# AntoineBlanot/LC2IS

Measured on AMD Instinct MI355X. Metric: training-step images/sec (512x512, ADE20K-150), higher is better.
Workload: dtype bf16; 1 GPU; BaseModelWithText ViT-B/16 + CLIP-text + decoder + fused head/CE train step, 512x512, 151 classes, text len 16, sgd; batch_per_gpu=32, global_batch=32, parallelism=dp1

## Files before the change

### include/lc2is_hip.h

```cpp
#ifndef LC2IS_HIP_H
#define LC2IS_HIP_H
#include <stddef.h>
#include <stdint.h>

#ifdef __cplusplus
extern "C" {
#endif

#define LC2IS_ACT_NONE 0
#define LC2IS_ACT_QUICK_GELU 1
#define LC2IS_ACT_RELU 2
#define LC2IS_ACT_DQUICK_GELU 3
#define LC2IS_ACT_DRELU 4
#define LC2IS_ACT_QUICK_GELU_GRAD 5
#define LC2IS_ACT_MUL_AUX 6
#define LC2IS_ACT_GELU_ERF 7
#define LC2IS_ACT_DGELU_ERF 8
#define LC2IS_ACT_ADD_AUX 9

#define LC2IS_INTERP_BICUBIC 0
#define LC2IS_INTERP_BILINEAR 1

typedef void* lc2is_stream_t;

typedef struct {
  const void* src;
  void* dst;
  void* dstT;
  int N, K, ld_dst, ld_dstT;
  int tile_start;
  int flags;
} lc2is_shadow_desc;

const char* lc2is_version(void);

int lc2is_set_cu_budget(int ncu);
int lc2is_get_cu_budget(void);

int lc2is_gemm_nt_bf16(const void* A, int lda, const void* W, int ldw, const float* bias,
                       const float* resid, int ldr, const void* aux_in, int ldx, void* out_bf16, int ldo,
                       float* out_f32, int ldf, void* aux_out, int ldy, int M, int N, int K, int act,
                       int tile_cfg, lc2is_stream_t stream);

size_t lc2is_gemm_nt_ln_xchg_bytes(int M, int N);
int lc2is_gemm_nt_ln_bf16(const void* A, int lda, const void* W, int ldw, const float* bias, const float* resid, int ldr,
                          float* out_f32, int ldf, const float* gamma, const float* beta, float eps, void* ln_out, int ldl,
                          float* mean, float* rstd, void* xchg, size_t xchg_bytes, int M, int N, int K, lc2is_stream_t stream);

int lc2is_gemm_nt_bf16_batched(const void* A, int lda, long stride_a, const void* W, int ldw, long stride_w,
                               void* out_bf16, int ldo, long stride_ob, float* out_f32, int ldf, long stride_of,
                               int M, int N, int K, int batch, lc2is_stream_t stream);

size_t lc2is_gemm_tn_workspace_bytes(int M, int N, int K);
int lc2is_gemm_tn_bf16(const void* dY, int ldy, const void* X, int ldx, float* dW, int ldw, float* db, int M,
                       int N, int K, int accumulate, void* workspace, size_t workspace_bytes,
                       lc2is_stream_t stream);

#define LC2IS_TN_GROUP_MAX 128
typedef struct lc2is_tn_problem {
  const void* dY; const void* X; float* dW; float* db;
  int ldy, ldx, ldw, M, N, K, accumulate;
} lc2is_tn_problem;
size_t lc2is_gemm_tn_grouped_workspace_bytes(const lc2is_tn_problem* problems, int n);
int lc2is_gemm_tn_grouped(const lc2is_tn_problem* problems, int n, void* workspace, size_t workspace_bytes,
                          lc2is_stream_t stream);
int lc2is_release_captured_tables(void);
int lc2is_captured_tables_mark(void);
int lc2is_release_captured_tables_range(int first, int last);

size_t lc2is_colsum_workspace_bytes(int M, int N);
int lc2is_colsum_bf16(const void* dY, int ldy, float* db, int M, int N, int accumulate, void* workspace,
                      size_t workspace_bytes, lc2is_stream_t stream);

int lc2is_layernorm_fwd(const void* x, int ldx, int x_is_bf16, const float* gamma, const float* beta, void* y_bf16,
                        int ldy, float* y_f32, int ldyf, float* mean, float* rstd, int M, int C, float eps,
                        lc2is_stream_t stream);

size_t lc2is_layernorm_bwd_workspace_bytes(int M, int C);
int lc2is_layernorm_bwd(const void* dy_bf16, int lddy, const float* dy_f32, int lddyf, const void* x,
                        int ldx, int x_is_bf16, const float* gamma, const float* mean, const float* rstd,
                        const void* dres, int lddres, int dres_is_bf16, float* dx_f32, int lddx, void* dx_bf16,
                        int lddxb, float* dgamma, float* dbeta, int accumulate, int M, int C, void* workspace,
                        size_t workspace_bytes, lc2is_stream_t stream);

#define LC2IS_LN_PARTIALS_MAX 64
typedef struct {
  const float* partials;
  float* dgamma;
  float* dbeta;
  int nparts;
  int C;
  int accumulate;
} lc2is_ln_partials;
int lc2is_layernorm_bwd_partials(int M, int C);
int lc2is_ln_partials_reduce(const lc2is_ln_partials* items, int n, lc2is_stream_t stream);

int lc2is_attention_fwd(const void* Q, int ldq, const void* K, int ldk, const void* V, int ldv, void* O,
                        int ldo, float* lse2, const float* kbias, int B, int H, int Sq, int Sk, int D,
                        float scale, int causal, lc2is_stream_t stream);

int lc2is_attention_bwd(const void* Q, int ldq, const void* K, int ldk, const void* V, int ldv,
                        const void* O, int ldo, const void* dO, int lddo, void* dQ, int lddq, void* dK,
                        int lddk, void* dV, int lddv, const float* lse2, float* delta, const float* kbias,
                        int B, int H, int Sq, int Sk, int D, float scale, int causal, lc2is_stream_t stream);

int lc2is_attention_fwd_dropout(const void* Q, int ldq, const void* K, int ldk, const void* V, int ldv, void* O,
                                int ldo, float* lse2, const float* kbias, int B, int H, int Sq, int Sk, int D,
                                float scale, int causal, float p_drop, unsigned long long seed, lc2is_stream_t stream);
int lc2is_attention_bwd_dropout(const void* Q, int ldq, const void* K, int ldk, const void* V, int ldv,
                                const void* O, int ldo, const void* dO, int lddo, void* dQ, int lddq, void* dK,
                                int lddk, void* dV, int lddv, const float* lse2, float* delta, const float* kbias,
                                int B, int H, int Sq, int Sk, int D, float scale, int causal, float p_drop,
                                unsigned long long seed, lc2is_stream_t stream);

int lc2is_dropout_rows_f32(const float* x, int ldx, const float* resid, int ldr, float* y32, int ldy, void* y16,
                           int ldy16, int M, int C, int rows_per_sample, float p, unsigned long long seed,
                           lc2is_stream_t stream);
int lc2is_dropout_rows_bf16(const void* x, int ldx, void* y, int ldy, int M, int C, float p, unsigned long long seed,
                            lc2is_stream_t stream);
int lc2is_dropout_mask(unsigned char* out, long rows, int cols, float p, unsigned long long seed, lc2is_stream_t stream);


int lc2is_shadow_refresh(const lc2is_shadow_desc* descs, int ndesc, int total_tiles, lc2is_stream_t stream);
int lc2is_cast_f32_bf16(const float* src, int ld_src, void* dst_bf16, int ld_dst, int M, int C,
                        lc2is_stream_t stream);
int lc2is_transpose_bf16(const void* src, int ld_src, void* dst, int ld_dst, int R, int C,
                         lc2is_stream_t stream);
int lc2is_transpose_bf16_batched(const void* src, int ld_src, long stride_src, void* dst, int ld_dst, long stride_dst,
                                 int R, int C, int batch, lc2is_stream_t stream);

int lc2is_patchify(const float* pixels, void* out_bf16, int ld_out, int B, int H, int W, int patch,
                   lc2is_stream_t stream);
int lc2is_vit_embed_fwd(const float* patch, int ld_patch, const float* cls, const float* pos, float* x,
                        int ldx, int B, int P, int C, lc2is_stream_t stream);
int lc2is_vit_embed_bwd(const float* dx, int ldx, float* dpos, float* dcls, void* dpatch_bf16, int ld_dpatch,
                        int B, int P, int C, int accumulate, lc2is_stream_t stream);
int lc2is_text_embed_fwd(const int64_t* ids, const float* tok, const float* pos, float* x, int ldx, int B,
                         int L, int C, int vocab, lc2is_stream_t stream);
int lc2is_text_embed_bwd(const int64_t* ids, const float* dx, int ldx, float* dtok, float* dpos, int B, int L,
                         int C, int vocab, int accumulate, lc2is_stream_t stream);
int lc2is_rows_copy_f32(const float* src, int S_src, int src_off, float* dst_f32, void* dst_bf16, int S_dst,
                        int dst_off, int B, int n, int C, lc2is_stream_t stream);
int lc2is_rows_copy_bf16(const void* src, int S_src, int src_off, float* dst_f32, void* dst_bf16, int S_dst,
                         int dst_off, int B, int n, int C, lc2is_stream_t stream);

int lc2is_sgd_step(float* params, const float* grads, float* momentum_buf, size_t n, float lr, float momentum,
                   float weight_decay, float grad_scale, lc2is_stream_t stream);
int lc2is_adamw_step(float* params, const float* grads, float* exp_avg, float* exp_avg_sq, size_t n, float lr,
                     float beta1, float beta2, float eps, float weight_decay, int step, float grad_scale,
                     lc2is_stream_t stream);

size_t lc2is_head_upsample_ce_workspace_bytes(int B, int h, int w, int C, int S, int mode, int want_grad);
int lc2is_head_upsample_ce(const float* scores_lo, int ld, const int64_t* labels, float* dscores_lo,
                           float* scores_hi, float* loss_sum, int B, int h, int w, int C, int S, int mode,
                           long ignore_index, float grad_scale, void* workspace, size_t workspace_bytes,
                           lc2is_stream_t stream);
int lc2is_head_upsample_ce_opts(const float* scores_lo, int ld, const int64_t* labels, float* dscores_lo,
                                float* scores_hi, float* loss_sum, int B, int h, int w, int C, int S, int mode,
                                long ignore_index, float grad_scale, const float* class_weight, float label_smoothing,
                                void* workspace, size_t workspace_bytes, lc2is_stream_t stream);
int lc2is_upsample_bwd_nchw(const float* dhi, float* dlo, int ld, int B, int h, int w, int C, int S, int mode,
                            lc2is_stream_t stream);
int lc2is_ce_nchw_fwd(const float* logits, const int64_t* labels, float* lse, float* loss_sum, int B, int C,
                      long HW, long ignore_index, lc2is_stream_t stream);
int lc2is_ce_nchw_bwd(const float* logits, const int64_t* labels, const float* lse, const float* grad_scale_dev,
                      float grad_scale, float* dlogits, int B, int C, long HW, long ignore_index,
                      lc2is_stream_t stream);
int lc2is_ce_nchw_fwd_opts(const float* logits, const int64_t* labels, float* lse, float* loss_sum, float* loss_px,
                           int B, int C, long HW, long ignore_index, const float* class_weight, float label_smoothing,
                           lc2is_stream_t stream);
int lc2is_ce_nchw_bwd_opts(const float* logits, const int64_t* labels, const float* lse, const float* grad_scale_dev,
                           float grad_scale, const float* grad_px, float* dlogits, int B, int C, long HW,
                           long ignore_index, const float* class_weight, float label_smoothing,
                           lc2is_stream_t stream);
size_t lc2is_ce_nchw_fwd_workspace_bytes(int B, long HW);
int lc2is_ce_nchw_fwd_ordered(const float* logits, const int64_t* labels, float* lse, float* loss_sum, float* loss_px,
                              int B, int C, long HW, long ignore_index, const float* class_weight, float label_smoothing,
// ... 139 lines not shown
```

### lc2is_amd/csrc/layernorm.hip

```cpp
#include "common.h"
#include "lc2is_hip.h"
#include <cstdlib>

namespace {

#ifndef LN_BWD_OCC
#define LN_BWD_OCC 4
#endif
constexpr int LN_MAXV = 8;

__device__ __forceinline__ float4 load_bf16x4(const bf16_t* p) {
  const uint2 pk = *reinterpret_cast<const uint2*>(p);
  return make_float4(bf16_to_f32((bf16_t)(pk.x & 0xffff)), bf16_to_f32((bf16_t)(pk.x >> 16)),
                     bf16_to_f32((bf16_t)(pk.y & 0xffff)), bf16_to_f32((bf16_t)(pk.y >> 16)));
}

template <int NV>
__global__ __launch_bounds__(256) void ln_fwd_kernel(const float* __restrict__ x, const bf16_t* __restrict__ xb, int ldx,
                                                      const float* __restrict__ gamma,
                                                      const float* __restrict__ beta, bf16_t* y, int ldy,
                                                      float* yf, int ldyf, float* mean_out, float* rstd_out,
                                                      int M, int C, float eps) {
  const int lane = threadIdx.x & 63;
  const int C4 = C >> 2;
  float4 gm[NV], bt[NV];
#pragma unroll
  for (int i = 0; i < NV; ++i) {
    const int c4 = lane + 64 * i;
    gm[i] = (c4 < C4) ? reinterpret_cast<const float4*>(gamma)[c4] : make_float4(0.f, 0.f, 0.f, 0.f);
    bt[i] = (beta && c4 < C4) ? reinterpret_cast<const float4*>(beta)[c4] : make_float4(0.f, 0.f, 0.f, 0.f);
  }
  const int stride = gridDim.x * 4;
  int row = blockIdx.x * 4 + (threadIdx.x >> 6);
  if (row >= M) return;
  auto load_row = [&](int r, float4 (&dst)[NV]) __attribute__((always_inline)) {
    if (xb) {
#pragma unroll
      for (int i = 0; i < NV; ++i) {
        const int c4 = lane + 64 * i;
        dst[i] = (c4 < C4) ? load_bf16x4(xb + (size_t)r * ldx + 4 * c4) : make_float4(0.f, 0.f, 0.f, 0.f);
      }
      return;
    }
    const float4* xr = reinterpret_cast<const float4*>(x + (size_t)r * ldx);
#pragma unroll
    for (int i = 0; i < NV; ++i) {
      const int c4 = lane + 64 * i;
      dst[i] = (c4 < C4) ? xr[c4] : make_float4(0.f, 0.f, 0.f, 0.f);
    }
  };
  float4 v[NV], nx[NV];
  load_row(row, v);
  for (; row < M; row += stride) {
    const bool more = row + stride < M;
    if (more) load_row(row + stride, nx);
    float s = 0.f;
#pragma unroll
    for (int i = 0; i < NV; ++i) {
      const int c4 = lane + 64 * i;
      if (c4 < C4) s += (v[i].x + v[i].y) + (v[i].z + v[i].w);
    }
    const float mean = wave_sum(s) / (float)C;
    float q = 0.f;
#pragma unroll
    for (int i = 0; i < NV; ++i) {
      const int c4 = lane + 64 * i;
      if (c4 < C4) {
        const float a = v[i].x - mean, b = v[i].y - mean, c = v[i].z - mean, d = v[i].w - mean;
        q += (a * a + b * b) + (c * c + d * d);
      }
    }
    const float rstd = rsqrtf(wave_sum(q) / (float)C + eps);
    if (lane == 0) {
      if (mean_out) mean_out[row] = mean;
      if (rstd_out) rstd_out[row] = rstd;
    }
#pragma unroll
    for (int i = 0; i < NV; ++i) {
      const int c4 = lane + 64 * i;
      if (c4 < C4) {
        float4 o;
        o.x = (v[i].x - mean) * rstd * gm[i].x;
        o.y = (v[i].y - mean) * rstd * gm[i].y;
        o.z = (v[i].z - mean) * rstd * gm[i].z;
// ... 123 lines not shown
    for (int c = threadIdx.x; c < 2 * C; c += 256) ws[(size_t)rz * 2 * C + c] = 0.f;
  float4 gm[NV], dg[NV], db[NV];
#pragma unroll
  for (int i = 0; i < NV; ++i) {
    const int c4 = lane + 64 * i;
    gm[i] = (c4 < C4) ? reinterpret_cast<const float4*>(gamma)[c4] : make_float4(0.f, 0.f, 0.f, 0.f);
    dg[i] = make_float4(0.f, 0.f, 0.f, 0.f);
    db[i] = make_float4(0.f, 0.f, 0.f, 0.f);
  }
  struct Raw { uint2 dy[NV], rv[NV]; f32x4_t xf[XB ? 1 : NV]; uint2 xb[XB ? NV : 1]; };
  auto load_row = [&](int row, Raw& r) __attribute__((always_inline)) {
#pragma unroll
    for (int i = 0; i < NV; ++i) {
      const int c4 = lane + 64 * i;
      const bool ok = c4 < C4;
      r.rv[i] = (dresb && ok) ? *reinterpret_cast<const uint2*>(dresb + (size_t)row * lddres + 4 * c4) : make_uint2(0u, 0u);
      r.dy[i] = ok ? *reinterpret_cast<const uint2*>(dyb + (size_t)row * lddy + 4 * c4) : make_uint2(0u, 0u);
      if constexpr (XB) r.xb[i] = ok ? *reinterpret_cast<const uint2*>((const bf16_t*)xv_ + (size_t)row * ldx + 4 * c4) : make_uint2(0u, 0u);
      else r.xf[i] = ok ? __builtin_nontemporal_load(reinterpret_cast<const f32x4_t*>((const float*)xv_ + (size_t)row * ldx + 4 * c4))
                        : f32x4_t{0.f, 0.f, 0.f, 0.f};
    }
  };
  auto widen = [](uint2 pk) {
    return make_float4(bf16_to_f32((bf16_t)(pk.x & 0xffff)), bf16_to_f32((bf16_t)(pk.x >> 16)),
                       bf16_to_f32((bf16_t)(pk.y & 0xffff)), bf16_to_f32((bf16_t)(pk.y >> 16)));
  };
  const int stride = gridDim.x * 4;
  int row = blockIdx.x * 4 + wave;
  Raw cur, nxt;
  if (row < M) load_row(row, cur);
  for (; row < M; row += stride) {
    const bool more = row + stride < M;
    if (more) load_row(row + stride, nxt);
    const float mu = mean[row], rs = rstd[row];
    float4 xh[NV], dy[NV];
    float s1 = 0.f, s2 = 0.f;
#pragma unroll
    for (int i = 0; i < NV; ++i) {
      const int c4 = lane + 64 * i;
      if (c4 < C4) {
        float4 xv;
        if constexpr (XB) xv = widen(cur.xb[i]);
        else xv = make_float4(cur.xf[i][0], cur.xf[i][1], cur.xf[i][2], cur.xf[i][3]);
        dy[i] = widen(cur.dy[i]);
        xh[i] = make_float4((xv.x - mu) * rs, (xv.y - mu) * rs, (xv.z - mu) * rs, (xv.w - mu) * rs);
        const float a = dy[i].x * gm[i].x, b = dy[i].y * gm[i].y, c = dy[i].z * gm[i].z, d = dy[i].w * gm[i].w;
        s1 += (a + b) + (c + d);
        s2 += (a * xh[i].x + b * xh[i].y) + (c * xh[i].z + d * xh[i].w);
        dg[i].x += dy[i].x * xh[i].x; dg[i].y += dy[i].y * xh[i].y;
        dg[i].z += dy[i].z * xh[i].z; dg[i].w += dy[i].w * xh[i].w;
        db[i].x += dy[i].x; db[i].y += dy[i].y; db[i].z += dy[i].z; db[i].w += dy[i].w;
      }
    }
    const float c1 = wave_sum(s1) / (float)C, c2 = wave_sum(s2) / (float)C;
#pragma unroll
    for (int i = 0; i < NV; ++i) {
      const int c4 = lane + 64 * i;
      if (c4 < C4) {
        const float4 rv = widen(cur.rv[i]);
        float4 o;
        o.x = rs * (dy[i].x * gm[i].x - c1 - xh[i].x * c2);
        o.y = rs * (dy[i].y * gm[i].y - c1 - xh[i].y * c2);
        o.z = rs * (dy[i].z * gm[i].z - c1 - xh[i].z * c2);
        o.w = rs * (dy[i].w * gm[i].w - c1 - xh[i].w * c2);
        o.x += rv.x; o.y += rv.y; o.z += rv.z; o.w += rv.w;
        uint2 pk = make_uint2(pack_bf16x2(o.x, o.y), pack_bf16x2(o.z, o.w));
        __builtin_nontemporal_store(i32x2_t{(int)pk.x, (int)pk.y}, reinterpret_cast<i32x2_t*>(dxb + (size_t)row * lddxb + 4 * c4));
      }
    }
    if (more) cur = nxt;
  }
  float* r = red;
#pragma unroll
  for (int pass = 0; pass < 2; ++pass) {
    __syncthreads();
#pragma unroll
    for (int i = 0; i < NV; ++i) {
      const int c4 = lane + 64 * i;
      if (c4 < C4) *reinterpret_cast<float4*>(r + wave * 2048 + 4 * c4) = pass ? db[i] : dg[i];
    }
    __syncthreads();
    for (int c = threadIdx.x; c < C; c += 256) {
      const float t = (r[c] + r[2048 + c]) + (r[4096 + c] + r[6144 + c]);
      ws[((size_t)blockIdx.x * 2 + pass) * C + c] = t;
    }
  }
}

__global__ __launch_bounds__(256) void ln_bwd_reduce_kernel(const float* __restrict__ ws, int nblk, int C,
                                                             float* dgamma, float* dbeta, int accumulate) {
  const int c = blockIdx.x * 256 + threadIdx.x;
  if (c >= C) return;
  float g = 0.f, b = 0.f;
  for (int k = 0; k < nblk; ++k) {
    g += ws[((size_t)k * 2 + 0) * C + c];
    b += ws[((size_t)k * 2 + 1) * C + c];
  }
  if (dgamma) dgamma[c] = accumulate ? dgamma[c] + g : g;
  if (dbeta) dbeta[c] = accumulate ? dbeta[c] + b : b;
}

inline int ln_bwd_blocks(int M, int C) {
  const int nv = (C / 4 + 63) / 64;
  const int cap = 256 * (nv <= 3 ? LN_BWD_OCC : nv == 4 ? 3 : nv <= 6 ? 2 : 1);
  int nb = (M + 3) / 4;
  return nb > cap ? cap : nb;
}

}

static int ln_fwd_blocks(int M) {
  static const int cap = getenv("LC2IS_LN_FWD_BLOCKS") ? atoi(getenv("LC2IS_LN_FWD_BLOCKS")) : 2048;
  const int need = (M + 3) / 4;
  return need < cap ? need : (cap > 0 ? cap : need);
}

extern "C" int lc2is_layernorm_fwd(const void* x, int ldx, int x_is_bf16, const float* gamma, const float* beta,
                                   void* y_bf16, int ldy, float* y_f32, int ldyf, float* mean, float* rstd,
                                   int M, int C, float eps, lc2is_stream_t stream_) {
  hipStream_t stream = (hipStream_t)stream_;
  if (!x || !gamma || (!y_bf16 && !y_f32)) return LC2IS_ERR_NULL;
  const float* xf = x_is_bf16 ? nullptr : (const float*)x;
  const bf16_t* xb = x_is_bf16 ? (const bf16_t*)x : nullptr;
  if (M <= 0 || C <= 0 || C % 4 || C > LN_MAXV * 256) return LC2IS_ERR_SHAPE;
  if (ldx < C || ldx % 4 || (y_bf16 && (ldy < C || ldy % 4)) || (y_f32 && (ldyf < C || ldyf % 4)))
    return LC2IS_ERR_SHAPE;
#define LN_FWD(NV_)                                                                                  \
  hipLaunchKernelGGL(ln_fwd_kernel<NV_>, dim3(ln_fwd_blocks(M)), dim3(256), 0, stream, xf, xb, ldx, gamma, beta, \
                     (bf16_t*)y_bf16, ldy, y_f32, ldyf, mean, rstd, M, C, eps)
  const int nv = (C / 4 + 63) / 64;
  if (nv <= 1) LN_FWD(1); else if (nv == 2) LN_FWD(2); else if (nv == 3) LN_FWD(3);
  else if (nv == 4) LN_FWD(4); else if (nv <= 6) LN_FWD(6); else LN_FWD(8);
#undef LN_FWD
  return lc2is_check_launch();
}

extern "C" size_t lc2is_layernorm_bwd_workspace_bytes(int M, int C) {
  if (M <= 0 || C <= 0) return 0;
  return (size_t)ln_bwd_blocks(M, C) * 2 * (size_t)C * sizeof(float);
}

extern "C" int lc2is_layernorm_bwd(const void* dy_bf16, int lddy, const float* dy_f32, int lddyf,
                                   const void* x, int ldx, int x_is_bf16, const float* gamma, const float* mean,
                                   const float* rstd, const void* dres, int lddres, int dres_is_bf16, float* dx_f32,
                                   int lddx, void* dx_bf16, int lddxb, float* dgamma, float* dbeta, int accumulate,
                                   int M, int C, void* workspace, size_t workspace_bytes,
                                   lc2is_stream_t stream_) {
  hipStream_t stream = (hipStream_t)stream_;
  const float* xf = x_is_bf16 ? nullptr : (const float*)x;
  const bf16_t* xb = x_is_bf16 ? (const bf16_t*)x : nullptr;
  const float* dresf = dres_is_bf16 ? nullptr : (const float*)dres;
  const bf16_t* dresb = dres_is_bf16 ? (const bf16_t*)dres : nullptr;
  if ((!dy_bf16 && !dy_f32) || !x || !gamma || !mean || !rstd || (!dx_f32 && !dx_bf16)) return LC2IS_ERR_NULL;
  if (M <= 0 || C <= 0 || C % 4 || C > LN_MAXV * 256) return LC2IS_ERR_SHAPE;
  if (ldx < C || ldx % 4) return LC2IS_ERR_SHAPE;
  if ((dy_f32 ? (lddyf < C || lddyf % 4) : (lddy < C || lddy % 4))) return LC2IS_ERR_SHAPE;
  if ((dres && (lddres < C || lddres % 4)) || (dx_f32 && (lddx < C || lddx % 4)) ||
      (dx_bf16 && (lddxb < C || lddxb % 4)))
    return LC2IS_ERR_SHAPE;
  if (!workspace || workspace_bytes < lc2is_layernorm_bwd_workspace_bytes(M, C)) return LC2IS_ERR_WORKSPACE;
  const int nblk = ln_bwd_blocks(M, C);
  const int nv = (C / 4 + 63) / 64;
  static const bool lean_on = !(getenv("LC2IS_LN_BWD_LEAN") && atoi(getenv("LC2IS_LN_BWD_LEAN")) == 0);
  if (lean_on && dy_bf16 && !dy_f32 && !dx_f32 && dx_bf16 && (!dres || dres_is_bf16) && nv <= 4) {
    const int cap = 256 * (nv <= 2 ? 4 : nv == 3 ? 3 : 2);
    const int lgrid = nblk < cap ? nblk : cap;
#define LN_LEAN(NV_)                                                                                                       \
  do {                                                                                                                     \
    if (x_is_bf16)                                                                                                         \
      hipLaunchKernelGGL((ln_bwd_lean_kernel<NV_, true>), dim3(lgrid), dim3(256), 0, stream, (const bf16_t*)dy_bf16, lddy, x, \
                         ldx, gamma, mean, rstd, (const bf16_t*)dres, lddres, (bf16_t*)dx_bf16, lddxb, (float*)workspace, nblk, M, C); \
    else                                                                                                                   \
      hipLaunchKernelGGL((ln_bwd_lean_kernel<NV_, false>), dim3(lgrid), dim3(256), 0, stream, (const bf16_t*)dy_bf16, lddy, x, \
                         ldx, gamma, mean, rstd, (const bf16_t*)dres, lddres, (bf16_t*)dx_bf16, lddxb, (float*)workspace, nblk, M, C); \
  } while (0)
    if (nv <= 1) LN_LEAN(1); else if (nv == 2) LN_LEAN(2); else if (nv == 3) LN_LEAN(3); else LN_LEAN(4);
#undef LN_LEAN
    int rc = lc2is_check_launch();
    if (rc) return rc;
    if (dgamma || dbeta) {
      hipLaunchKernelGGL(partials_reduce_kernel, dim3((C + 31) / 32, 2), dim3(1024), 0, stream,
                         (const float*)workspace, nblk, (size_t)2 * C, (size_t)C, C, dgamma, dbeta, accumulate);
      rc = lc2is_check_launch();
    }
    return rc;
  }
#define LN_BWD(NV_)                                                                                   \
  hipLaunchKernelGGL(ln_bwd_kernel<NV_>, dim3(nblk), dim3(256), 0, stream, (const bf16_t*)dy_bf16, lddy, \
                     dy_f32, lddyf, xf, xb, ldx, gamma, mean, rstd, dresf, dresb, lddres, dx_f32, lddx,  \
                     (bf16_t*)dx_bf16, lddxb, (float*)workspace, M, C)
  if (nv <= 1) LN_BWD(1); else if (nv == 2) LN_BWD(2); else if (nv == 3) LN_BWD(3);
  else if (nv == 4) LN_BWD(4); else if (nv <= 6) LN_BWD(6); else LN_BWD(8);
#undef LN_BWD
  int rc = lc2is_check_launch();
  if (rc) return rc;
  if (dgamma || dbeta) {
    hipLaunchKernelGGL(partials_reduce_kernel, dim3((C + 31) / 32, 2), dim3(1024), 0, stream,
                       (const float*)workspace, nblk, (size_t)2 * C, (size_t)C, C, dgamma, dbeta, accumulate);
    rc = lc2is_check_launch();
  }
  return rc;
}

extern "C" int lc2is_layernorm_bwd_partials(int M, int C) {
  if (M <= 0 || C <= 0 || C % 4 || C > LN_MAXV * 256) return 0;
  return ln_bwd_blocks(M, C);
}

namespace {
struct LnPartialsGroup {
  lc2is_ln_partials item[LC2IS_LN_PARTIALS_MAX];
};
__global__ __launch_bounds__(1024) void ln_partials_reduce_grouped_kernel(LnPartialsGroup g) {
  const lc2is_ln_partials& it = g.item[blockIdx.z];
  if ((int)blockIdx.x * 32 >= it.C) return;
  float* out = blockIdx.y ? it.dbeta : it.dgamma;
  if (!out) return;
  partials_reduce_body(it.partials + (size_t)blockIdx.y * it.C, it.nparts, (size_t)2 * it.C, it.C, out, it.accumulate,
                       blockIdx.x);
}
}

extern "C" int lc2is_ln_partials_reduce(const lc2is_ln_partials* items, int n, lc2is_stream_t stream_) {
  hipStream_t stream = (hipStream_t)stream_;
  if (!items) return LC2IS_ERR_NULL;
  if (n <= 0 || n > LC2IS_LN_PARTIALS_MAX) return LC2IS_ERR_SHAPE;
  LnPartialsGroup g{};
  int cmax = 0;
  for (int i = 0; i < n; ++i) {
    const lc2is_ln_partials& it = items[i];
    if (!it.partials || (!it.dgamma && !it.dbeta)) return LC2IS_ERR_NULL;
    if (it.nparts <= 0 || it.C <= 0 || it.C % 4) return LC2IS_ERR_SHAPE;
    for (int j = 0; j < i; ++j)
      if ((it.dgamma && (it.dgamma == items[j].dgamma || it.dgamma == items[j].dbeta)) ||
          (it.dbeta && (it.dbeta == items[j].dgamma || it.dbeta == items[j].dbeta)))
        return LC2IS_ERR_UNSUPPORTED;
    g.item[i] = it;
    cmax = it.C > cmax ? it.C : cmax;
  }
  hipLaunchKernelGGL(ln_partials_reduce_grouped_kernel, dim3((cmax + 31) / 32, 2, n), dim3(1024), 0, stream, g);
  return lc2is_check_launch();
}
```

### lc2is_amd/ops.py

```python
from __future__ import annotations

import ctypes as C
import os

import torch

from . import _lib

ACT_NONE, ACT_QUICK_GELU, ACT_RELU, ACT_DQUICK_GELU, ACT_DRELU, ACT_QUICK_GELU_GRAD, ACT_MUL_AUX = 0, 1, 2, 3, 4, 5, 6
ACT_GELU_ERF, ACT_DGELU_ERF, ACT_ADD_AUX = 7, 8, 9

_P, _I, _F, _Z, _L, _U64 = C.c_void_p, C.c_int, C.c_float, C.c_size_t, C.c_long, C.c_ulonglong
_ARGTYPES = {
    "lc2is_gemm_nt_bf16": [_P, _I, _P, _I, _P, _P, _I, _P, _I, _P, _I, _P, _I, _P, _I, _I, _I, _I, _I, _I, _P],
    "lc2is_gemm_nt_ln_xchg_bytes": [_I, _I],
    "lc2is_gemm_nt_ln_bf16": [_P, _I, _P, _I, _P, _P, _I, _P, _I, _P, _P, _F, _P, _I, _P, _P, _P, _Z, _I, _I, _I, _P],
    "lc2is_gemm_nt_bf16_batched": [_P, _I, _L, _P, _I, _L, _P, _I, _L, _P, _I, _L, _I, _I, _I, _I, _P],
    "lc2is_transpose_bf16_batched": [_P, _I, _L, _P, _I, _L, _I, _I, _I, _P],
    "lc2is_gemm_tn_workspace_bytes": [_I, _I, _I],
    "lc2is_gemm_tn_bf16": [_P, _I, _P, _I, _P, _I, _P, _I, _I, _I, _I, _P, _Z, _P],
    "lc2is_colsum_workspace_bytes": [_I, _I],
    "lc2is_colsum_bf16": [_P, _I, _P, _I, _I, _I, _P, _Z, _P],
    "lc2is_layernorm_fwd": [_P, _I, _I, _P, _P, _P, _I, _P, _I, _P, _P, _I, _I, _F, _P],
    "lc2is_layernorm_bwd_partials": [_I, _I],
    "lc2is_ln_partials_reduce": [_P, _I, _P],
    "lc2is_layernorm_bwd_workspace_bytes": [_I, _I],
    "lc2is_layernorm_bwd": [_P, _I, _P, _I, _P, _I, _I, _P, _P, _P, _P, _I, _I, _P, _I, _P, _I, _P, _P, _I, _I, _I,
                            _P, _Z, _P],
    "lc2is_attention_fwd": [_P, _I, _P, _I, _P, _I, _P, _I, _P, _P, _I, _I, _I, _I, _I, _F, _I, _P],
    "lc2is_attention_bwd": [_P, _I, _P, _I, _P, _I, _P, _I, _P, _I, _P, _I, _P, _I, _P, _I, _P, _P, _P,
                            _I, _I, _I, _I, _I, _F, _I, _P],
    "lc2is_attention_fwd_dropout": [_P, _I, _P, _I, _P, _I, _P, _I, _P, _P, _I, _I, _I, _I, _I, _F, _I, _F, _U64, _P],
    "lc2is_attention_bwd_dropout": [_P, _I, _P, _I, _P, _I, _P, _I, _P, _I, _P, _I, _P, _I, _P, _I, _P, _P, _P,
                                    _I, _I, _I, _I, _I, _F, _I, _F, _U64, _P],
    "lc2is_dropout_rows_f32": [_P, _I, _P, _I, _P, _I, _P, _I, _I, _I, _I, _F, _U64, _P],
    "lc2is_dropout_rows_bf16": [_P, _I, _P, _I, _I, _I, _F, _U64, _P],
    "lc2is_dropout_mask": [_P, _L, _I, _F, _U64, _P],
    "lc2is_shadow_refresh": [_P, _I, _I, _P],
    "lc2is_set_cu_budget": [_I],
    "lc2is_get_cu_budget": [],
    "lc2is_cast_f32_bf16": [_P, _I, _P, _I, _I, _I, _P],
    "lc2is_transpose_bf16": [_P, _I, _P, _I, _I, _I, _P],
    "lc2is_patchify": [_P, _P, _I, _I, _I, _I, _I, _P],
    "lc2is_vit_embed_fwd": [_P, _I, _P, _P, _P, _I, _I, _I, _I, _P],
    "lc2is_vit_embed_bwd": [_P, _I, _P, _P, _P, _I, _I, _I, _I, _I, _P],
    "lc2is_text_embed_fwd": [_P, _P, _P, _P, _I, _I, _I, _I, _I, _P],
    "lc2is_text_embed_bwd": [_P, _P, _I, _P, _P, _I, _I, _I, _I, _I, _P],
    "lc2is_rows_copy_bf16": [_P, _I, _I, _P, _P, _I, _I, _I, _I, _I, _P],
    "lc2is_rows_copy_f32": [_P, _I, _I, _P, _P, _I, _I, _I, _I, _I, _P],
    "lc2is_sgd_step": [_P, _P, _P, _Z, _F, _F, _F, _F, _P],
    "lc2is_adamw_step": [_P, _P, _P, _P, _Z, _F, _F, _F, _F, _F, _I, _F, _P],
    "lc2is_grad_sumsq_blocks": [_Z],
    "lc2is_grad_sumsq_workspace_bytes": [_Z],
    "lc2is_grad_sumsq": [_P, _Z, _P, _Z, _P],
    "lc2is_optim_ctrl_update": [_P, _P, _P, _I, _P, _I, _F, _F, _I, _F, _F, _P],
    "lc2is_sgd_step_ctrl": [_P, _P, _P, _Z, _P, _F, _F, _I, _P],
    "lc2is_adamw_step_ctrl": [_P, _P, _P, _P, _Z, _P, _F, _F, _F, _F, _I, _P],
    "lc2is_sgd_step_groups": [_P, _P, _P, _Z, _P, _P, _P, _I, _F, _I, _P],
    "lc2is_adamw_step_groups": [_P, _P, _P, _P, _Z, _P, _P, _P, _I, _F, _F, _F, _I, _P],
    "lc2is_head_upsample_ce_workspace_bytes": [_I, _I, _I, _I, _I, _I, _I],
    "lc2is_head_upsample_ce": [_P, _I, _P, _P, _P, _P, _I, _I, _I, _I, _I, _I, C.c_long, _F, _P, _Z, _P],
    "lc2is_ce_nchw_fwd": [_P, _P, _P, _P, _I, _I, C.c_long, C.c_long, _P],
    "lc2is_ce_nchw_bwd": [_P, _P, _P, _P, _F, _P, _I, _I, C.c_long, C.c_long, _P],
    "lc2is_head_upsample_ce_opts": [_P, _I, _P, _P, _P, _P, _I, _I, _I, _I, _I, _I, C.c_long, _F, _P, _F, _P, _Z, _P],
    "lc2is_ce_nchw_fwd_opts": [_P, _P, _P, _P, _P, _I, _I, C.c_long, C.c_long, _P, _F, _P],
    "lc2is_ce_nchw_fwd_workspace_bytes": [_I, C.c_long],
    "lc2is_ce_nchw_fwd_ordered": [_P, _P, _P, _P, _P, _I, _I, C.c_long, C.c_long, _P, _F, _P, _Z, _P],
    "lc2is_ce_nchw_bwd_opts": [_P, _P, _P, _P, _F, _P, _P, _I, _I, C.c_long, C.c_long, _P, _F, _P],
    "lc2is_upsample_bwd_nchw": [_P, _P, _I, _I, _I, _I, _I, _I, _I, _P],
    "lc2is_bilinear_up_fwd": [_P, _P, _P, _I, _I, _I, _I, _I, _P],
    "lc2is_bilinear_up_bwd": [_P, _P, _P, _I, _I, _I, _I, _I, _I, _P],
    "lc2is_sr_gather": [_P, _P, _I, _I, _I, _I, _I, _P],
    "lc2is_sr_scatter_add_f32": [_P, _P, _I, _I, _I, _I, _P],
    "lc2is_l2norm_fwd": [_P, _P, _P, _P, _I, _I, _F, _P],
    "lc2is_l2norm_bwd": [_P, _P, _P, _P, _I, _I, _F, _P],
    "lc2is_add_n": [_P, _P, _P, _P, _P, _P, _Z, _P],
    "lc2is_rows_ce": [_P, _P, _P, _P, _P, _F, _I, _I, _I, _P],
    "lc2is_cols_ce": [_P, _P, _P, _P, _F, _I, _I, _I, _I, _P],
    "lc2is_npair": [_P, _P, _P, _P, _I, _I, _I, _I, _P],
    "lc2is_miou_counts": [_P, _P, _P, _I, _I, _I, _I, _I, _P],
    "lc2is_resize_argmax_workspace_bytes": [_L, _I],
    "lc2is_resize_argmax": [_P, _I, _I, _I, _I, _I, _P, _L, _L, _P, _I, _P, _P, _P, _Z, _P],
    "lc2is_npair_bwd": [_P, _P, _P, _P, _P, _P, _P, _P, _I, _I, _I, _I, _P],
    "lc2is_gemm_tn_grouped_workspace_bytes": [_P, _I],
    "lc2is_gemm_tn_grouped": [_P, _I, _P, _Z, _P],
    "lc2is_release_captured_tables": [],
    "lc2is_captured_tables_mark": [],
    "lc2is_release_captured_tables_range": [_I, _I],
    "lc2is_rows_gather": [_P, _I, _I, _P, _I, _I, _P, _P, _I, _I, _I, _P],
    "lc2is_resample_u8": [_P, _I, _I, _I, _P, _I, _I, _P, _P, _I, _P],
    "lc2is_gather2d_u8": [_P, _I, _I, _I, _P, _I, _I, _P, _P, _P],
    "lc2is_crop_lut": [_P, _I, _I, _I, _I, _I, _I, _P, _P, _P, _P, _P],
    "lc2is_aug_params": [_P, _P, _I, _P, _P, _L, _P, _P, _P],
    "lc2is_aug_apply": [_P, _Z, _P, _Z, _P, _L, _P, _P, _I, _I, _I, _P, _L, _P, _P, _P],
    "lc2is_swin_attn_fwd": [_P, _I, _P, _I, _P, _P, _I, _I, _I, _I, _I, _I, _I, _I, _I, _F, _P],
    "lc2is_swin_bias_table_grad": [_P, _P, _P, _P, _I, _I, _I, _I, _P],
    "lc2is_swin_attn_bwd_workspace_bytes": [_I, _I, _I],
    "lc2is_swin_attn_bwd": [_P, _I, _P, _I, _P, _I, _P, _P, _P, _I, _P, _I, _I, _I, _I, _I, _I, _I, _I, _I, _I, _F,
                            _P, _Z, _P],
}
_bound = {}


def _fn(name: str):
    f = _bound.get(name)
    if f is None:
        f = getattr(_lib.load(), name)
        if name in _ARGTYPES:
            f.argtypes = _ARGTYPES[name]
        if name.endswith("_workspace_bytes"):
            f.restype = C.c_size_t
        _bound[name] = f
    return f


def _stream() -> int:
    return torch.cuda.current_stream().cuda_stream


def _chk(t: torch.Tensor | None, dtype, name: str, ndim: int | None = 2):
    if t is None:
        return
    if not t.is_cuda:
        raise RuntimeError(f"lc2is_amd: {name} must be a CUDA(HIP) tensor; there is no CPU path")
    if t.dtype != dtype:
        raise RuntimeError(f"lc2is_amd: {name} must be {dtype}, got {t.dtype}")
    if ndim is not None and t.dim() != ndim:
        raise RuntimeError(f"lc2is_amd: {name} must be {ndim}-D, got shape {tuple(t.shape)}")
    if t.dim() >= 1 and t.stride(-1) != 1:
        raise RuntimeError(f"lc2is_amd: {name} must have unit stride in its last dimension")


def _ptr(t: torch.Tensor | None) -> int | None:
    return None if t is None else t.data_ptr()


def _ld(t: torch.Tensor | None) -> int:
    return 0 if t is None else (t.stride(0) if t.dim() == 2 else t.shape[-1])


def _out(spec, shape, dtype, dev):
    if spec is True:
        return torch.empty(shape, dtype=dtype, device=dev)
    if spec is None or spec is False:
        return None
    return spec



_ws_cache: dict = {}


def workspace(nbytes: int, device, tag: str = "default") -> torch.Tensor:
    key = (str(device), _stream(), tag)
    buf = _ws_cache.get(key)
    if buf is None or buf.numel() < nbytes:
        buf = torch.empty(max(int(nbytes), 1 << 20), dtype=torch.uint8, device=device)
        _ws_cache[key] = buf
    return buf


def gemm_nt(a: torch.Tensor, w: torch.Tensor, bias: torch.Tensor | None = None, *, act: int = ACT_NONE,
            resid: torch.Tensor | None = None, aux_in: torch.Tensor | None = None,
            out_bf16: torch.Tensor | bool | None = True, out_f32: torch.Tensor | bool | None = None,
            aux_out: torch.Tensor | bool | None = None, tile_cfg: int = 0):
    _chk(a, torch.bfloat16, "a"); _chk(w, torch.bfloat16, "w")
    if resid is not None and resid.dtype == torch.bfloat16:
        if act != ACT_NONE or aux_in is not None:
            raise RuntimeError("lc2is_amd.gemm_nt: a bf16 residual needs act == ACT_NONE and no aux_in")
        act, aux_in, resid = ACT_ADD_AUX, resid, None
    _chk(bias, torch.float32, "bias", 1); _chk(resid, torch.float32, "resid"); _chk(aux_in, torch.bfloat16, "aux_in")
    M, K = a.shape
    N, K2 = w.shape
    if K2 != K:
        raise RuntimeError(f"lc2is_amd.gemm_nt: K mismatch {K} vs {K2}")
    if bias is not None and bias.numel() != N:
        raise RuntimeError("lc2is_amd.gemm_nt: bias length != N")
    dev = a.device
    ob = _out(out_bf16, (M, N), torch.bfloat16, dev)
    of = _out(out_f32, (M, N), torch.float32, dev)
    ao = _out(aux_out, (M, N), torch.bfloat16, dev)
    _chk(ob, torch.bfloat16, "out_bf16"); _chk(of, torch.float32, "out_f32"); _chk(ao, torch.bfloat16, "aux_out")
    rc = _fn("lc2is_gemm_nt_bf16")(_ptr(a), _ld(a), _ptr(w), _ld(w), _ptr(bias), _ptr(resid), _ld(resid),
                                   _ptr(aux_in), _ld(aux_in), _ptr(ob), _ld(ob), _ptr(of), _ld(of), _ptr(ao),
                                   _ld(ao), M, N, K, act, tile_cfg, _stream())
    _lib.check(rc, f"gemm_nt M={M} N={N} K={K}")
    return ob, of, ao


_xchg_cache = {}
_LN_FUSE = os.environ.get("LC2IS_LN_FUSE", "1") != "0"
_LN_FUSE_MIN_ROWS = int(os.environ.get("LC2IS_LN_FUSE_MIN_ROWS", "0"))

# ... 105 lines not shown
        _chk(dy, torch.bfloat16, "dy"); _chk(x, torch.bfloat16, "x"); _chk(dw, torch.float32, "dw"); _chk(db, torch.float32, "db", 1)
        M, N = dy.shape
        if x.shape[0] != M or tuple(dw.shape) != (N, x.shape[1]) or (db is not None and db.numel() != N):
            raise RuntimeError("lc2is_amd.gemm_tn_grouped: shape mismatch")
        arr[i] = TnProblem(_ptr(dy), _ptr(x), _ptr(dw), _ptr(db), _ld(dy), _ld(x), _ld(dw), M, N, x.shape[1], int(acc))
    nbytes = _fn("lc2is_gemm_tn_grouped_workspace_bytes")(arr, len(problems))
    ws = workspace(nbytes, problems[0][0].device, "gemm_tn_grouped")
    rc = _fn("lc2is_gemm_tn_grouped")(arr, len(problems), _ptr(ws), ws.numel(), _stream())
    _lib.check(rc, f"gemm_tn_grouped n={len(problems)}")


def release_captured_tables() -> int:
    f = _fn("lc2is_release_captured_tables")
    f.restype = C.c_int
    return int(f())


def captured_tables_mark() -> int:
    return int(_fn("lc2is_captured_tables_mark")())


def release_captured_tables_range(first: int, last: int) -> int:
    return int(_fn("lc2is_release_captured_tables_range")(int(first), int(last)))


def colsum(dy: torch.Tensor, db: torch.Tensor | None = None, accumulate: bool = False):
    _chk(dy, torch.bfloat16, "dy")
    M, N = dy.shape
    if db is None:
        db = torch.empty((N,), dtype=torch.float32, device=dy.device)
        accumulate = False
    _chk(db, torch.float32, "db", 1)
    nbytes = _fn("lc2is_colsum_workspace_bytes")(M, N)
    ws = workspace(nbytes, dy.device, "colsum")
    rc = _fn("lc2is_colsum_bf16")(_ptr(dy), _ld(dy), _ptr(db), M, N, int(accumulate), _ptr(ws), ws.numel(),
                                  _stream())
    _lib.check(rc, f"colsum M={M} N={N}")
    return db


def layernorm_fwd(x: torch.Tensor, gamma: torch.Tensor, beta: torch.Tensor | None, eps: float = 1e-5, *,
                  save_stats: bool = True, out_bf16: torch.Tensor | bool | None = True,
                  out_f32: torch.Tensor | bool | None = None):
    xb = x.dtype == torch.bfloat16
    _chk(x, torch.bfloat16 if xb else torch.float32, "x"); _chk(gamma, torch.float32, "gamma", 1); _chk(beta, torch.float32, "beta", 1)
    M, Cc = x.shape
    dev = x.device
    yb = _out(out_bf16, (M, Cc), torch.bfloat16, dev)
    yf = _out(out_f32, (M, Cc), torch.float32, dev)
    mean = torch.empty((M,), dtype=torch.float32, device=dev) if save_stats else None
    rstd = torch.empty((M,), dtype=torch.float32, device=dev) if save_stats else None
    rc = _fn("lc2is_layernorm_fwd")(_ptr(x), _ld(x), int(xb), _ptr(gamma), _ptr(beta), _ptr(yb), _ld(yb), _ptr(yf),
                                    _ld(yf), _ptr(mean), _ptr(rstd), M, Cc, float(eps), _stream())
    _lib.check(rc, f"layernorm_fwd M={M} C={Cc}")
    return yb, yf, mean, rstd


def layernorm_bwd(dy: torch.Tensor, x: torch.Tensor, gamma: torch.Tensor, mean: torch.Tensor,
                  rstd: torch.Tensor, *, dres: torch.Tensor | None = None, dgamma: torch.Tensor | None = None,
                  dbeta: torch.Tensor | None = None, accumulate: bool = False, want_f32: bool = True,
                  want_bf16: bool = True, need_param_grads: bool = True):
    M, Cc = x.shape
    dev = x.device
    dyb = dy if dy.dtype == torch.bfloat16 else None
    dyf = dy if dy.dtype == torch.float32 else None
    if dyb is None and dyf is None:
        raise RuntimeError("lc2is_amd.layernorm_bwd: dy must be bf16 or fp32")
    xb = x.dtype == torch.bfloat16
    rb = dres is not None and dres.dtype == torch.bfloat16
    _chk(dyb, torch.bfloat16, "dy"); _chk(dyf, torch.float32, "dy"); _chk(x, torch.bfloat16 if xb else torch.float32, "x")
    _chk(dres, torch.bfloat16 if rb else torch.float32, "dres")
    dxf = torch.empty((M, Cc), dtype=torch.float32, device=dev) if want_f32 else None
    dxb = torch.empty((M, Cc), dtype=torch.bfloat16, device=dev) if want_bf16 else None
    if need_param_grads:
        if dgamma is None:
            dgamma = torch.empty((Cc,), dtype=torch.float32, device=dev)
            accumulate = False
            if dbeta is None:
                dbeta = torch.empty((Cc,), dtype=torch.float32, device=dev)
    nbytes = _fn("lc2is_layernorm_bwd_workspace_bytes")(M, Cc)
    defer = _ln_defer if (need_param_grads and (dgamma is not None or dbeta is not None)) else None
    if defer is not None:
        ws = torch.empty(max(int(nbytes), 16), dtype=torch.uint8, device=dev)
        defer.append((ws, _fn("lc2is_layernorm_bwd_partials")(M, Cc), Cc, dgamma, dbeta, bool(accumulate)))
        pg, pb = None, None
    else:
        ws = workspace(nbytes, dev, "ln_bwd")
        pg, pb = dgamma, dbeta
    rc = _fn("lc2is_layernorm_bwd")(_ptr(dyb), _ld(dyb), _ptr(dyf), _ld(dyf), _ptr(x), _ld(x), int(xb), _ptr(gamma),
                                    _ptr(mean), _ptr(rstd), _ptr(dres), _ld(dres), int(rb), _ptr(dxf), _ld(dxf),
                                    _ptr(dxb), _ld(dxb), _ptr(pg), _ptr(pb), int(accumulate), M, Cc,
                                    _ptr(ws), ws.numel(), _stream())
    _lib.check(rc, f"layernorm_bwd M={M} C={Cc}")
    return dxf, dxb, dgamma, dbeta


class LnPartials(C.Structure):
    _fields_ = [("partials", C.c_void_p), ("dgamma", C.c_void_p), ("dbeta", C.c_void_p), ("nparts", C.c_int),
                ("C", C.c_int), ("accumulate", C.c_int)]


LN_PARTIALS_MAX = 64
_LN_DEFER = os.environ.get("LC2IS_LN_DEFER", "1") != "0"
_ln_defer = None


def ln_defer_begin():
    global _ln_defer
    prev, _ln_defer = _ln_defer, ([] if _LN_DEFER else None)
    return prev


def ln_defer_flush():
    global _ln_defer
    items = _ln_defer
    if not items:
        return
    _ln_defer = []
    while items:
        chunk, rest, seen = [], [], set()
        for it in items:
            outs = {t.data_ptr() for t in (it[3], it[4]) if t is not None}
            if len(chunk) < LN_PARTIALS_MAX and not (outs & seen) and not rest:
                chunk.append(it); seen |= outs
            else:
                rest.append(it)
        arr = (LnPartials * len(chunk))()
        for i, (ws, nparts, Cc, dg, db, acc) in enumerate(chunk):
            _chk(dg, torch.float32, "dgamma", 1); _chk(db, torch.float32, "dbeta", 1)
            arr[i] = LnPartials(_ptr(ws), _ptr(dg), _ptr(db), nparts, Cc, int(acc))
        rc = _fn("lc2is_ln_partials_reduce")(arr, len(chunk), _stream())
        _lib.check(rc, f"ln_partials_reduce n={len(chunk)}")
        items = rest


def ln_defer_end(prev):
    global _ln_defer
    ln_defer_flush()
    _ln_defer = prev


def attention_fwd(q: torch.Tensor, k: torch.Tensor, v: torch.Tensor, B: int, H: int, Sq: int, Sk: int, D: int,
                  scale: float, *, causal: bool = False, kbias: torch.Tensor | None = None,
                  save_lse: bool = True, out: torch.Tensor | None = None, dropout_p: float = 0.0, seed: int = 0):
    _chk(q, torch.bfloat16, "q"); _chk(k, torch.bfloat16, "k"); _chk(v, torch.bfloat16, "v")
    _chk(kbias, torch.float32, "kbias")
    if q.shape != (B * Sq, H * D) or k.shape != (B * Sk, H * D) or v.shape != (B * Sk, H * D):
        raise RuntimeError("lc2is_amd.attention_fwd: q/k/v shapes do not match B,H,S,D")
    if kbias is not None and (kbias.shape != (B, Sk) or not kbias.is_contiguous()):
        raise RuntimeError("lc2is_amd.attention_fwd: kbias must be contiguous [B,Sk]")
    o = out if out is not None else torch.empty((B * Sq, H * D), dtype=torch.bfloat16, device=q.device)
    _chk(o, torch.bfloat16, "out")
    lse = torch.empty((B, H, Sq), dtype=torch.float32, device=q.device) if save_lse else None
    if dropout_p > 0.0:
        rc = _fn("lc2is_attention_fwd_dropout")(_ptr(q), _ld(q), _ptr(k), _ld(k), _ptr(v), _ld(v), _ptr(o), _ld(o),
                                                _ptr(lse), _ptr(kbias), B, H, Sq, Sk, D, float(scale), int(causal),
                                                float(dropout_p), int(seed), _stream())
    else:
        rc = _fn("lc2is_attention_fwd")(_ptr(q), _ld(q), _ptr(k), _ld(k), _ptr(v), _ld(v), _ptr(o), _ld(o),
                                        _ptr(lse), _ptr(kbias), B, H, Sq, Sk, D, float(scale), int(causal),
                                        _stream())
    _lib.check(rc, f"attention_fwd B={B} H={H} Sq={Sq} Sk={Sk} D={D}")
    return o, lse


def attention_bwd(q, k, v, o, do, lse2, B: int, H: int, Sq: int, Sk: int, D: int, scale: float, *,
                  causal: bool = False, kbias: torch.Tensor | None = None, dq=None, dk=None, dv=None,
                  dropout_p: float = 0.0, seed: int = 0):
    for t, n in ((q, "q"), (k, "k"), (v, "v"), (o, "o"), (do, "do")):
        _chk(t, torch.bfloat16, n)
    _chk(lse2, torch.float32, "lse2", 3); _chk(kbias, torch.float32, "kbias")
    dev = q.device
    dq = dq if dq is not None else torch.empty((B * Sq, H * D), dtype=torch.bfloat16, device=dev)
    dk = dk if dk is not None else torch.empty((B * Sk, H * D), dtype=torch.bfloat16, device=dev)
    dv = dv if dv is not None else torch.empty((B * Sk, H * D), dtype=torch.bfloat16, device=dev)
    for t, n in ((dq, "dq"), (dk, "dk"), (dv, "dv")):
# ... 770 lines not shown
```

Before: 1051 images/s.

## Add two-rows-per-wave LayerNorm backward kernel for C=768 behind env flag

Adds a specialized LayerNorm backward kernel for C=768 with fp32 x and bf16 dy. Each wave processes two rows at once using 16-byte vector loads, shuffles and wave reductions, prefetches the next row pair, and caches gamma in shared memory. The lean path's partial count is now the launched grid size rather than nblk, and the count is exposed so the deferred partials reduction sums only the rows actually written. The new kernel runs only when LC2IS_LN_BWD_WIDE=1, so the default path gains only the smaller partial-count reduction.

```diff
diff --git a/include/lc2is_hip.h b/include/lc2is_hip.h
--- a/include/lc2is_hip.h
+++ b/include/lc2is_hip.h
@@ -93,6 +93,7 @@
   int accumulate;
 } lc2is_ln_partials;
 int lc2is_layernorm_bwd_partials(int M, int C);
+int lc2is_layernorm_bwd_rows_written(void);
 int lc2is_ln_partials_reduce(const lc2is_ln_partials* items, int n, lc2is_stream_t stream);
 
 int lc2is_attention_fwd(const void* Q, int ldq, const void* K, int ldk, const void* V, int ldv, void* O,
diff --git a/lc2is_amd/csrc/layernorm.hip b/lc2is_amd/csrc/layernorm.hip
--- a/lc2is_amd/csrc/layernorm.hip
+++ b/lc2is_amd/csrc/layernorm.hip
@@ -1,5 +1,6 @@
 #include "common.h"
 #include "lc2is_hip.h"
+#include <cstdint>
 #include <cstdlib>
 
 namespace {
@@ -289,6 +290,155 @@
     __syncthreads();
     for (int c = threadIdx.x; c < C; c += 256) {
       const float t = (r[c] + r[2048 + c]) + (r[4096 + c] + r[6144 + c]);
+      ws[((size_t)blockIdx.x * 2 + pass) * C + c] = t;
+    }
+  }
+}
+
+__device__ __forceinline__ float ln_rounded(float v) {
+  asm("" : "+v"(v));
+  return v;
+}
+__device__ __forceinline__ void ln_bwd_quad_sums(const float* d, const float* xq, f32x4_t gq, float& q1, float& q2) {
+  const float a = ln_rounded(d[0] * gq[0]), b = ln_rounded(d[1] * gq[1]), c = ln_rounded(d[2] * gq[2]), e = ln_rounded(d[3] * gq[3]);
+  q1 = (a + b) + (c + e);
+  q2 = (ln_rounded(a * xq[0]) + ln_rounded(b * xq[1])) + (ln_rounded(c * xq[2]) + ln_rounded(e * xq[3]));
+}
+__device__ __forceinline__ float ln_bwd_dx(float dy, float gm, float xh, float c1, float c2, float rs, float rv) {
+  return __builtin_fmaf(rs, __builtin_fmaf(-c2, xh, __builtin_fmaf(dy, gm, -c1)), rv);
+}
+
+#ifndef LN_BWD_WIDE_OCC
+#define LN_BWD_WIDE_OCC 2
+#endif
+__global__ __launch_bounds__(256, LN_BWD_WIDE_OCC) void ln_bwd_wide768_kernel(const bf16_t* __restrict__ dyb, int lddy,
+                                                      const float* __restrict__ x, int ldx,
+                                                      const float* __restrict__ gamma,
+                                                      const float* __restrict__ mean,
+                                                      const float* __restrict__ rstd,
+                                                      const bf16_t* __restrict__ dresb, int lddres,
+                                                      bf16_t* dxb, int lddxb, float* ws, int M) {
+  constexpr int C = 768;
+  __shared__ float red[2 * 4 * C];
+  const int lane = threadIdx.x & 63, wave = threadIdx.x >> 6;
+  const bool lo = lane < 32;
+  const int col[3] = {8 * lane, lo ? 512 + 8 * lane : 8 * (lane - 32), 256 + 8 * lane};
+  __shared__ __attribute__((aligned(16))) float gsm[C];
+  for (int c = threadIdx.x; c < C; c += 256) gsm[c] = gamma[c];
+  __syncthreads();
+  float dg[3][8], db[3][8];
+#pragma unroll
+  for (int k = 0; k < 3; ++k)
+#pragma unroll
+    for (int j = 0; j < 8; ++j) dg[k][j] = db[k][j] = 0.f;
+  struct Raw { i32x4_t dy[3], rv[3]; f32x4_t xf[3][2]; };
+  auto load_pair = [&](int pair, Raw& r) __attribute__((always_inline)) {
+    const int rowA = 2 * pair, rowB = rowA + 1;
+    const int rows[3] = {rowA, lo ? rowA : rowB, rowB};
+#pragma unroll
+    for (int k = 0; k < 3; ++k) {
+      const bool ok = rows[k] < M;
+      const size_t row = (size_t)rows[k];
+      r.rv[k] = (dresb && ok) ? *reinterpret_cast<const i32x4_t*>(dresb + row * lddres + col[k]) : i32x4_t{0, 0, 0, 0};
+      r.dy[k] = ok ? *reinterpret_cast<const i32x4_t*>(dyb + row * lddy + col[k]) : i32x4_t{0, 0, 0, 0};
+#pragma unroll
+      for (int h = 0; h < 2; ++h)
+        r.xf[k][h] = ok ? __builtin_nontemporal_load(reinterpret_cast<const f32x4_t*>(x + row * ldx + col[k] + 4 * h))
+                        : f32x4_t{0.f, 0.f, 0.f, 0.f};
+    }
+  };
+  const int npairs = (M + 1) >> 1;
+  const int stride = gridDim.x * 4;
+  int pair = blockIdx.x * 4 + wave;
+  const int hsrc = lane >> 1;
+  const bool odd = lane & 1;
+  Raw cur, nxt;
+  if (pair < npairs) load_pair(pair, cur);
+  for (; pair < npairs; pair += stride) {
+    const bool more = pair + stride < npairs;
+    if (more) load_pair(pair + stride, nxt);
+    const int rowA = 2 * pair, rowB = rowA + 1;
+    const bool hasB = rowB < M;
+    const float muA = mean[rowA], rsA = rstd[rowA];
+    const float muB = hasB ? mean[rowB] : 0.f, rsB = hasB ? rstd[rowB] : 0.f;
+    const float mu[3] = {muA, lo ? muA : muB, muB}, rs[3] = {rsA, lo ? rsA : rsB, rsB};
+    float dy[3][8], xh[3][8], q1[3][2], q2[3][2];
+#pragma unroll
+    for (int k = 0; k < 3; ++k) {
+#pragma unroll
+      for (int w = 0; w < 4; ++w) {
+        const unsigned pk = (unsigned)cur.dy[k][w];
+        dy[k][2 * w] = bf16_to_f32((bf16_t)(pk & 0xffff));
+        dy[k][2 * w + 1] = bf16_to_f32((bf16_t)(pk >> 16));
+      }
+#pragma unroll
+      for (int h = 0; h < 2; ++h) {
+        float* d = dy[k] + 4 * h;
+        float* xq = xh[k] + 4 * h;
+        const f32x4_t gq = *reinterpret_cast<const f32x4_t*>(gsm + col[k] + 4 * h);
+#pragma unroll
+        for (int j = 0; j < 4; ++j) xq[j] = (cur.xf[k][h][j] - mu[k]) * rs[k];
+        ln_bwd_quad_sums(d, xq, gq, q1[k][h], q2[k][h]);
+#pragma unroll
+        for (int j = 0; j < 4; ++j) {
+          dg[k][4 * h + j] = __builtin_fmaf(xq[j], d[j], dg[k][4 * h + j]);
+          db[k][4 * h + j] += d[j];
+        }
+      }
+    }
+    auto fetch = [&](const float (&q)[2], int src) __attribute__((always_inline)) {
+      const float t0 = __shfl(q[0], src, 64), t1 = __shfl(q[1], src, 64);
+      return odd ? t1 : t0;
+    };
+    float s1A = 0.f, s2A = 0.f, s1B = 0.f, s2B = 0.f;
+    s1A += fetch(q1[0], hsrc); s1A += fetch(q1[0], 32 + hsrc); s1A += fetch(q1[1], hsrc);
+    s2A += fetch(q2[0], hsrc); s2A += fetch(q2[0], 32 + hsrc); s2A += fetch(q2[1], hsrc);
+    s1B += fetch(q1[1], 32 + hsrc); s1B += fetch(q1[2], hsrc); s1B += fetch(q1[2], 32 + hsrc);
+    s2B += fetch(q2[1], 32 + hsrc); s2B += fetch(q2[2], hsrc); s2B += fetch(q2[2], 32 + hsrc);
+    const float c1A = wave_sum(s1A) / (float)C, c2A = wave_sum(s2A) / (float)C;
+    const float c1B = wave_sum(s1B) / (float)C, c2B = wave_sum(s2B) / (float)C;
+    const float c1[3] = {c1A, lo ? c1A : c1B, c1B}, c2[3] = {c2A, lo ? c2A : c2B, c2B};
+    const int rows[3] = {rowA, lo ? rowA : rowB, rowB};
+#pragma unroll
+    for (int k = 0; k < 3; ++k) {
+      float o[8], gm[8];
+#pragma unroll
+      for (int h = 0; h < 2; ++h) {
+        const f32x4_t gq = *reinterpret_cast<const f32x4_t*>(gsm + col[k] + 4 * h);
+#pragma unroll
+        for (int j = 0; j < 4; ++j) gm[4 * h + j] = gq[j];
+      }
+#pragma unroll
+      for (int w = 0; w < 4; ++w) {
+        const unsigned pk = (unsigned)cur.rv[k][w];
+        const float r0 = bf16_to_f32((bf16_t)(pk & 0xffff)), r1 = bf16_to_f32((bf16_t)(pk >> 16));
+        o[2 * w] = ln_bwd_dx(dy[k][2 * w], gm[2 * w], xh[k][2 * w], c1[k], c2[k], rs[k], r0);
+        o[2 * w + 1] = ln_bwd_dx(dy[k][2 * w + 1], gm[2 * w + 1], xh[k][2 * w + 1], c1[k], c2[k], rs[k], r1);
+      }
+      if (rows[k] < M) {
+        const i32x4_t pk = {(int)pack_bf16x2(o[0], o[1]), (int)pack_bf16x2(o[2], o[3]), (int)pack_bf16x2(o[4], o[5]),
+                            (int)pack_bf16x2(o[6], o[7])};
+        __builtin_nontemporal_store(pk, reinterpret_cast<i32x4_t*>(dxb + (size_t)rows[k] * lddxb + col[k]));
+      }
+    }
+    if (more) cur = nxt;
+  }
+  const int slot[3] = {0, lo ? 0 : 1, 1};
+#pragma unroll
+  for (int pass = 0; pass < 2; ++pass) {
+    __syncthreads();
+#pragma unroll
+    for (int k = 0; k < 3; ++k) {
+      const float* s = pass ? db[k] : dg[k];
+      float* dst = red + (slot[k] * 4 + wave) * C + col[k];
+      *reinterpret_cast<float4*>(dst) = make_float4(s[0], s[1], s[2], s[3]);
+      *reinterpret_cast<float4*>(dst + 4) = make_float4(s[4], s[5], s[6], s[7]);
+    }
+    __syncthreads();
+    for (int c = threadIdx.x; c < C; c += 256) {
+      const float* ra = red + c;
+      const float* rb = red + 4 * C + c;
+      const float t = ((ra[0] + rb[0]) + (ra[C] + rb[C])) + ((ra[2 * C] + rb[2 * C]) + (ra[3 * C] + rb[3 * C]));
       ws[((size_t)blockIdx.x * 2 + pass) * C + c] = t;
     }
   }
@@ -346,6 +496,9 @@
   if (M <= 0 || C <= 0) return 0;
   return (size_t)ln_bwd_blocks(M, C) * 2 * (size_t)C * sizeof(float);
 }
+
+static thread_local int g_ln_bwd_rows_written = 0;
+extern "C" int lc2is_layernorm_bwd_rows_written(void) { return g_ln_bwd_rows_written; }
 
 extern "C" int lc2is_layernorm_bwd(const void* dy_bf16, int lddy, const float* dy_f32, int lddyf,
                                    const void* x, int ldx, int x_is_bf16, const float* gamma, const float* mean,
@@ -369,29 +522,42 @@
   const int nblk = ln_bwd_blocks(M, C);
   const int nv = (C / 4 + 63) / 64;
   static const bool lean_on = !(getenv("LC2IS_LN_BWD_LEAN") && atoi(getenv("LC2IS_LN_BWD_LEAN")) == 0);
+  static const bool wide_on = getenv("LC2IS_LN_BWD_WIDE") && atoi(getenv("LC2IS_LN_BWD_WIDE")) == 1;
   if (lean_on && dy_bf16 && !dy_f32 && !dx_f32 && dx_bf16 && (!dres || dres_is_bf16) && nv <= 4) {
+    int rc;
+    int lgrid;
+    if (wide_on && C == 768 && !x_is_bf16 && lddy % 8 == 0 && lddxb % 8 == 0 && (!dres || lddres % 8 == 0) &&
+        (((uintptr_t)dy_bf16 | (uintptr_t)dx_bf16 | (uintptr_t)dres | (uintptr_t)x | (uintptr_t)gamma) & 15) == 0) {
+      const int need = ((M + 1) / 2 + 3) / 4;
+      lgrid = need < 256 * LN_BWD_WIDE_OCC ? need : 256 * LN_BWD_WIDE_OCC;
+      hipLaunchKernelGGL(ln_bwd_wide768_kernel, dim3(lgrid), dim3(256), 0, stream, (const bf16_t*)dy_bf16, lddy, xf, ldx, gamma,
+                         mean, rstd, (const bf16_t*)dres, lddres, (bf16_t*)dx_bf16, lddxb, (float*)workspace, M);
+    } else {
     const int cap = 256 * (nv <= 2 ? 4 : nv == 3 ? 3 : 2);
-    const int lgrid = nblk < cap ? nblk : cap;
+    lgrid = nblk < cap ? nblk : cap;
 #define LN_LEAN(NV_)                                                                                                       \
   do {                                                                                                                     \
     if (x_is_bf16)                                                                                                         \
       hipLaunchKernelGGL((ln_bwd_lean_kernel<NV_, true>), dim3(lgrid), dim3(256), 0, stream, (const bf16_t*)dy_bf16, lddy, x, \
-                         ldx, gamma, mean, rstd, (const bf16_t*)dres, lddres, (bf16_t*)dx_bf16, lddxb, (float*)workspace, nblk, M, C); \
+                         ldx, gamma, mean, rstd, (const bf16_t*)dres, lddres, (bf16_t*)dx_bf16, lddxb, (float*)workspace, lgrid, M, C); \
     else                                                                                                                   \
       hipLaunchKernelGGL((ln_bwd_lean_kernel<NV_, false>), dim3(lgrid), dim3(256), 0, stream, (const bf16_t*)dy_bf16, lddy, x, \
-                         ldx, gamma, mean, rstd, (const bf16_t*)dres, lddres, (bf16_t*)dx_bf16, lddxb, (float*)workspace, nblk, M, C); \
+                         ldx, gamma, mean, rstd, (const bf16_t*)dres, lddres, (bf16_t*)dx_bf16, lddxb, (float*)workspace, lgrid, M, C); \
   } while (0)
     if (nv <= 1) LN_LEAN(1); else if (nv == 2) LN_LEAN(2); else if (nv == 3) LN_LEAN(3); else LN_LEAN(4);
 #undef LN_LEAN
-    int rc = lc2is_check_launch();
+    }
+    g_ln_bwd_rows_written = lgrid;
+    rc = lc2is_check_launch();
     if (rc) return rc;
     if (dgamma || dbeta) {
       hipLaunchKernelGGL(partials_reduce_kernel, dim3((C + 31) / 32, 2), dim3(1024), 0, stream,
-                         (const float*)workspace, nblk, (size_t)2 * C, (size_t)C, C, dgamma, dbeta, accumulate);
+                         (const float*)workspace, lgrid, (size_t)2 * C, (size_t)C, C, dgamma, dbeta, accumulate);
       rc = lc2is_check_launch();
     }
     return rc;
   }
+  g_ln_bwd_rows_written = nblk;
 #define LN_BWD(NV_)                                                                                   \
   hipLaunchKernelGGL(ln_bwd_kernel<NV_>, dim3(nblk), dim3(256), 0, stream, (const bf16_t*)dy_bf16, lddy, \
                      dy_f32, lddyf, xf, xb, ldx, gamma, mean, rstd, dresf, dresb, lddres, dx_f32, lddx,  \
diff --git a/lc2is_amd/ops.py b/lc2is_amd/ops.py
--- a/lc2is_amd/ops.py
+++ b/lc2is_amd/ops.py
@@ -23,6 +23,7 @@
     "lc2is_colsum_bf16": [_P, _I, _P, _I, _I, _I, _P, _Z, _P],
     "lc2is_layernorm_fwd": [_P, _I, _I, _P, _P, _P, _I, _P, _I, _P, _P, _I, _I, _F, _P],
     "lc2is_layernorm_bwd_partials": [_I, _I],
+    "lc2is_layernorm_bwd_rows_written": [],
     "lc2is_ln_partials_reduce": [_P, _I, _P],
     "lc2is_layernorm_bwd_workspace_bytes": [_I, _I],
     "lc2is_layernorm_bwd": [_P, _I, _P, _I, _P, _I, _I, _P, _P, _P, _P, _I, _I, _P, _I, _P, _I, _P, _P, _I, _I, _I,
@@ -108,7 +109,7 @@
         f = getattr(_lib.load(), name)
         if name in _ARGTYPES:
             f.argtypes = _ARGTYPES[name]
-        if name.endswith("_workspace_bytes"):
+        if name.endswith("_workspace_bytes") or name.endswith("_xchg_bytes"):
             f.restype = C.c_size_t
         _bound[name] = f
     return f
@@ -380,7 +381,6 @@
     defer = _ln_defer if (need_param_grads and (dgamma is not None or dbeta is not None)) else None
     if defer is not None:
         ws = torch.empty(max(int(nbytes), 16), dtype=torch.uint8, device=dev)
-        defer.append((ws, _fn("lc2is_layernorm_bwd_partials")(M, Cc), Cc, dgamma, dbeta, bool(accumulate)))
         pg, pb = None, None
     else:
         ws = workspace(nbytes, dev, "ln_bwd")
@@ -390,6 +390,8 @@
                                     _ptr(dxb), _ld(dxb), _ptr(pg), _ptr(pb), int(accumulate), M, Cc,
                                     _ptr(ws), ws.numel(), _stream())
     _lib.check(rc, f"layernorm_bwd M={M} C={Cc}")
+    if defer is not None:
+        defer.append((ws, _fn("lc2is_layernorm_bwd_rows_written")(), Cc, dgamma, dbeta, bool(accumulate)))
     return dxf, dxb, dgamma, dbeta
 
 
```

New measurement: 1049 images/s. No clear change (-0.1%).
